# loicmagne/tinynerf

Measured on AMD Instinct MI355X. Metric: ray-samples/sec (K-Planes training step: sampler + render fwd + bwd + Adam), higher is better.
Workload: dtype f32 (f16x2-split products)

## Files before the change

tinynerf_amd/csrc/mlp_wgrad_rc.hip:

```cpp
#include "mlp_stage.h"
#include "mlp_f2_heads.h"
#include "b3_device.h"
#include "phase_timers.h"
#include <algorithm>

#ifndef TN_RC_SB
#define TN_RC_SB
#endif
TN_PHASE_COUNTERS(tn_phase_cycles_rc, tn_debug_phase_cycles_rc)
#define TN_PTR_BEGIN TN_PHASE_BEGIN(ptr_)
#define TN_PTR(k) TN_PHASE(tn_phase_cycles_rc, ptr_, k)
namespace {

using tn::f32x16;
using tn::f32x4;
using namespace tn::mlp;
namespace b3 = tn::b3;

constexpr int H = 64, NH = 4;

template <int CTRL>
__device__ __forceinline__ float dpp_max(float v) {
    return fmaxf(v, __int_as_float(__builtin_amdgcn_update_dpp(0, __float_as_int(v), CTRL, 0xf, 0xf, true)));
}
__device__ __forceinline__ float wave_max(float m) {
    m = dpp_max<0xB1>(m);
    m = dpp_max<0x4E>(m);
    m = dpp_max<0x141>(m);
    m = dpp_max<0x128>(m);
    const auto r16 = __builtin_amdgcn_permlane16_swap(__float_as_uint(m), __float_as_uint(m), false, false);
    m = fmaxf(__uint_as_float(r16[0]), __uint_as_float(r16[1]));
    const auto r32 = __builtin_amdgcn_permlane32_swap(__float_as_uint(m), __float_as_uint(m), false, false);
    return fmaxf(__uint_as_float(r32[0]), __uint_as_float(r32[1]));
}

__device__ __forceinline__ void load_block_f(const float *__restrict__ rows, int i, int h, float (&v)[16]) {
    const f32x4 *p = reinterpret_cast<const f32x4 *>(rows + i * 32 + 4 * h);
#pragma unroll
    for (int q = 0; q < 4; ++q) {
        const f32x4 t = p[2 * q];
        v[4 * q] = t[0]; v[4 * q + 1] = t[1]; v[4 * q + 2] = t[2]; v[4 * q + 3] = t[3];
    }
}

__device__ __forceinline__ void split_block(const float (&v)[16], b3::Op (&op)[2]) {
    const float a[8] = {v[0], v[1], v[2], v[3], v[4], v[5], v[6], v[7]};
    const float b[8] = {v[8], v[9], v[10], v[11], v[12], v[13], v[14], v[15]};
    op[0] = b3::split8(a);
    op[1] = b3::split8(b);
}

struct WOp { u32x4h a0h, a0l, a1h, a1l; };
__device__ __forceinline__ WOp load_w(const _Float16 *__restrict__ Wh, int plane, int stride, int j, int h, int b) {
    const _Float16 *p0 = Wh + j * stride + 16 * b + 8 * h, *p1 = p0 + 32 * stride;
    WOp w;
    w.a0h = *reinterpret_cast<const u32x4h *>(p0); w.a0l = *reinterpret_cast<const u32x4h *>(p0 + plane);
    w.a1h = *reinterpret_cast<const u32x4h *>(p1); w.a1l = *reinterpret_cast<const u32x4h *>(p1 + plane);
    return w;
}
template <bool S>
__device__ __forceinline__ void mma_sf(const WOp &w, const u32x4h &bh, const u32x4h &bl, f32x16 (&accS)[2], f32x16 (&accF)[2], bool first = false) {
    const f32x16 z = {0.f, 0.f, 0.f, 0.f, 0.f, 0.f, 0.f, 0.f, 0.f, 0.f, 0.f, 0.f, 0.f, 0.f, 0.f, 0.f};
    if constexpr (S) {
        accS[0] = mfma_f16(w.a0l, bh, first ? z : accS[0]);
        accS[1] = mfma_f16(w.a1l, bh, first ? z : accS[1]);
    }
    accF[0] = mfma_f16(bh, w.a0l, first ? z : accF[0]);
    accF[1] = mfma_f16(bh, w.a1l, first ? z : accF[1]);
    if constexpr (S) {
        accS[0] = mfma_f16(w.a0h, bl, accS[0]);
        accS[1] = mfma_f16(w.a1h, bl, accS[1]);
    }
    accF[0] = mfma_f16(bl, w.a0h, accF[0]);
    accF[1] = mfma_f16(bl, w.a1h, accF[1]);
    if constexpr (S) {
        accS[0] = mfma_f16(w.a0h, bh, accS[0]);
        accS[1] = mfma_f16(w.a1h, bh, accS[1]);
    }
    accF[0] = mfma_f16(bh, w.a0h, accF[0]);
    accF[1] = mfma_f16(bh, w.a1h, accF[1]);
}

struct RcArgs {
    MlpArgs a, b;
    const float *x, *aux;
    const float *ws_a, *ws_b;
    float *gW[5], *gB[5];
    float *gWs, *gBs;
    int64_t n;
};

template <int WPB, bool AUX, int OA, int OB, int NGA, int NBA>
__device__ __forceinline__ void wgrad_rc_body(const RcArgs &p, const float *__restrict__ ldsa, const float *__restrict__ ldsb, float *__restrict__ ,
                                              const float *__restrict__ px, const float *__restrict__ paux, const int *__restrict__ paidx,
                                              const float *__restrict__ pws_a, const float *__restrict__ pws_b)
{
    const int lane = tn::lane_id(), j_ = lane & 31, h_ = lane >> 5;
    const int wave = __builtin_amdgcn_readfirstlane(threadIdx.x >> 6);
    const int64_t n = p.n, n_tiles = (n + 31) >> 5;
    const int Rta = StashTile(H, NH, 0).rows(), Rtb = StashTile(H, 1, 0).rows();
    constexpr int nga = NGA, nba = NBA;
    constexpr bool has_aux = AUX;

    f32x16 acc[3][2][2];
#pragma unroll
    for (int l = 0; l < 3; ++l)
#pragma unroll
        for (int tn_ = 0; tn_ < 2; ++tn_)
#pragma unroll
            for (int tk = 0; tk < 2; ++tk)
#pragma unroll
                for (int r = 0; r < 16; ++r) acc[l][tn_][tk][r] = 0.0f;
    float db[3][2] = {{0.f, 0.f}, {0.f, 0.f}, {0.f, 0.f}};
    float dwo[OA][2], dws[OB][2], dbo[OA], dbs[OB];
#pragma unroll
    for (int o = 0; o < OA; ++o) { dwo[o][0] = dwo[o][1] = 0.f; dbo[o] = 0.f; }
#pragma unroll
    for (int o = 0; o < OB; ++o) { dws[o][0] = dws[o][1] = 0.f; dbs[o] = 0.f; }

    f32x4 fr[12], av[8];
    auto fetch_x = [&](int64_t t) {
        int64_t r = t * 32 + j_;
        r = r < n ? r : n - 1;
        const float *xr = px + r * 96 + 4 * h_;
#pragma unroll
        for (int g = 0; g < 12; ++g) fr[g] = *reinterpret_cast<const f32x4 *>(xr + 8 * g);
    };
    int aidx = 0;
    auto fetch_aidx = [&](int64_t t) {
        int64_t r = t * 32 + j_;
        r = r < n ? r : n - 1;
        if constexpr (has_aux) aidx = paidx[r];
    };
    auto fetch_aux = [&]() {
        if constexpr (has_aux) {
            const float *arow = paux + (int64_t)aidx * p.a.aux_stride + 4 * h_;
#pragma unroll
            for (int g = 0; g < 8; ++g) av[g] = *reinterpret_cast<const f32x4 *>(arow + 8 * (g < nga ? g : nga - 1));
        }
    };
    {
        const int64_t t0 = (int64_t)blockIdx.x * WPB + wave;
        fetch_aidx(t0 < n_tiles ? t0 : n_tiles - 1);
        fetch_aux();
        fetch_x(t0 < n_tiles ? t0 : n_tiles - 1);
    }
    float gqa[2][16], gqb[2][16];
    for (int64_t tile = (int64_t)blockIdx.x * WPB + wave; tile < n_tiles; tile += (int64_t)gridDim.x * WPB) {
        int j = j_, h = h_;
        asm volatile("" : "+v"(j), "+v"(h));
        const float *wsa = pws_a + tile * (int64_t)(Rta * 32);
        const float *wsb = pws_b + tile * (int64_t)(Rtb * 32);
        const _Float16 *W0 = reinterpret_cast<const _Float16 *>(ldsa + p.a.w_off[0]);
        const int plane0 = p.a.f2_plane[0], st0 = p.a.stride[0];
        const int64_t tile_next = tile + (int64_t)gridDim.x * WPB < n_tiles ? tile + (int64_t)gridDim.x * WPB : n_tiles - 1;
        fetch_aidx(tile_next);
        TN_PTR_BEGIN

        f32x16 accS[2], accF[2], actS[2], actF[2];
        if constexpr (has_aux) {
            WOp w = load_w(W0, plane0, st0, j, h, 6);
            float m = 0.0f;
#pragma unroll
            for (int g = 0; g < 8; ++g) m = tn::max_abs4(m, av[g]);
            float s_a, inv_a;
            f2_scales(wave_max(m), s_a, inv_a);
#pragma unroll
            for (int ba = 0; ba < nba; ++ba) {
                const WOp wn = load_w(W0, plane0, st0, j, h, 6 + (ba + 1 < nba ? ba + 1 : ba));
                const float v[8] = {av[2 * ba][0], av[2 * ba][1], av[2 * ba][2], av[2 * ba][3], av[2 * ba + 1][0], av[2 * ba + 1][1], av[2 * ba + 1][2], av[2 * ba + 1][3]};
                u32x4h bh, bl;
                f2_split8(v, s_a, bh, bl);
                mma_sf<true>(w, bh, bl, accS, accF, ba == 0);
                TN_RC_SB
                w = wn;
            }
            const float ca = inv_a * ldsa[p.a.f2_scale + 1];
#pragma unroll
            for (int ob = 0; ob < 2; ++ob) {
#pragma unroll
                for (int r = 0; r < 16; ++r) { actS[ob][r] = accS[ob][r] * ca; actF[ob][r] = accF[ob][r] * ca; }
            }
        } else {
            tn::zero_tiles(actS); tn::zero_tiles(actF);
        }
        TN_RC_SB
        TN_PTR(0)
        u32x4h xbh[6], xbl[6];
        float inv_x;
        {
            float m = 0.0f;
#pragma unroll
            for (int g = 0; g < 12; ++g) m = tn::max_abs4(m, fr[g]);
            float s_x;
            f2_scales(wave_max(m), s_x, inv_x);
#pragma unroll
            for (int b = 0; b < 6; ++b) {
                const float v[8] = {fr[2 * b][0], fr[2 * b][1], fr[2 * b][2], fr[2 * b][3], fr[2 * b + 1][0], fr[2 * b + 1][1], fr[2 * b + 1][2], fr[2 * b + 1][3]};
                f2_split8(v, s_x, xbh[b], xbl[b]);
            }
        }
        TN_RC_SB
        TN_PTR(1)
        load_block_f(wsa + (int64_t)((NH + 1) * H) * 32, j, h, gqa[0]);
        load_block_f(wsa + (int64_t)((NH + 1) * H + 32) * 32, j, h, gqa[1]);
        {
            WOp w = load_w(W0, plane0, st0, j, h, 0);
#pragma unroll
            for (int b = 0; b < 6; ++b) {
                const WOp wn = load_w(W0, plane0, st0, j, h, b + 1 < 6 ? b + 1 : b);
                mma_sf<true>(w, xbh[b], xbl[b], accS, accF, b == 0);
                TN_RC_SB
                w = wn;
            }
            const float cx = inv_x * ldsa[p.a.f2_scale + 1];
#pragma unroll
            for (int ob = 0; ob < 2; ++ob) {
                const f32x16 bias = tn::bias_tile(ldsa + p.a.b_off[0], ob, h);
                const float bl_ = ldsa[p.a.b_off[0] + 32 * ob + j];
#pragma unroll
                for (int r = 0; r < 16; ++r) {
                    actS[ob][r] = fmaf(accS[ob][r], cx, actS[ob][r]) + bias[r];
                    actF[ob][r] = fmaf(accF[ob][r], cx, actF[ob][r]) + bl_;
                }
                actS[ob] = tn::relu16(actS[ob]);
                actF[ob] = tn::relu16(actF[ob]);
            }
        }
        TN_RC_SB
        TN_PTR(2)
        {
            const _Float16 *W0s = reinterpret_cast<const _Float16 *>(ldsb + p.b.w_off[0]);
            const int pls = p.b.f2_plane[0], sts = p.b.stride[0];
            float gs[OB][16];
#pragma unroll
            for (int o = 0; o < OB; ++o) load_block_f(wsb + 2 * H * 32, o, h, gs[o]);
            WOp w = load_w(W0s, pls, sts, j, h, 0);
#pragma unroll
            for (int b = 0; b < 6; ++b) {
                const WOp wn = load_w(W0s, pls, sts, j, h, b + 1 < 6 ? b + 1 : b);
                mma_sf<false>(w, xbh[b], xbl[b], accS, accF, b == 0);
                TN_RC_SB
                w = wn;
            }
            const float c = inv_x * ldsb[p.b.f2_scale + 1];
#pragma unroll
            for (int ob = 0; ob < 2; ++ob) {
                const float bias = ldsb[p.b.b_off[0] + 32 * ob + j];
#pragma unroll
                for (int r = 0; r < 16; ++r) accF[ob][r] = fmaf(accF[ob][r], c, bias);
                accF[ob] = tn::relu16(accF[ob]);
            }
#pragma unroll
            for (int o = 0; o < OB; ++o) {
                float s0 = 0.f, s1 = 0.f, sg = 0.f;
#pragma unroll
                for (int r = 0; r < 16; ++r) { s0 = fmaf(gs[o][r], accF[0][r], s0); s1 = fmaf(gs[o][r], accF[1][r], s1); sg += gs[o][r]; }
                dws[o][0] += s0; dws[o][1] += s1; dbs[o] += sg;
            }
        }
        TN_RC_SB
        TN_PTR(3)

        float go[OA][16];
#pragma unroll
        for (int l = 1; l <= 3; ++l) {
            const _Float16 *Wl = reinterpret_cast<const _Float16 *>(ldsa + p.a.w_off[l]);
            const int plane = p.a.f2_plane[l], stride = p.a.stride[l];
            float (&gq)[2][16] = (l == 2) ? gqb : gqa;
            if (l < 3) {
                float (&gn)[2][16] = (l == 1) ? gqb : gqa;
                load_block_f(wsa + (int64_t)((NH + l + 1) * H) * 32, j, h, gn[0]);
                load_block_f(wsa + (int64_t)((NH + l + 1) * H + 32) * 32, j, h, gn[1]);
            }
            {
                b3::Op HB[2][2];
#pragma unroll
                for (int tk = 0; tk < 2; ++tk) {
                    float v[16];
#pragma unroll
                    for (int r = 0; r < 16; ++r) v[r] = actF[tk][r];
                    split_block(v, HB[tk]);
                }
#pragma unroll
                for (int tn_ = 0; tn_ < 2; ++tn_) {
                    float sg = 0.f;
#pragma unroll
                    for (int r = 0; r < 16; ++r) sg += gq[tn_][r];
                    db[l - 1][tn_] += sg;
                    b3::Op GA[2];
                    split_block(gq[tn_], GA);
#pragma unroll
                    for (int c = 0; c < 2; ++c)
#pragma unroll
                        for (int tk = 0; tk < 2; ++tk) acc[l - 1][tn_][tk] = b3::mfma6(GA[c], HB[tk][c], acc[l - 1][tn_][tk]);
                    TN_RC_SB
                }
            }
            TN_PTR(3 + l)
            if (l == 1) fetch_aux();
            if (l == 3) {
#pragma unroll
                for (int o = 0; o < OA; ++o) load_block_f(wsa + 2 * NH * H * 32, o, h, go[o]);
                fetch_x(tile_next);
            }
            WOp w = load_w(Wl, plane, stride, j, h, 0);
            float m = 0.0f;
#pragma unroll
            for (int kb = 0; kb < 2; ++kb)
#pragma unroll
                for (int r = 0; r < 16; ++r) m = fmaxf(m, actS[kb][r]);
            float s, inv;
            f2_scales(wave_max(m), s, inv);
#pragma unroll
            for (int b = 0; b < 4; ++b) {
                const WOp wn = load_w(Wl, plane, stride, j, h, b + 1 < 4 ? b + 1 : b);
                float v[8];
#pragma unroll
                for (int e = 0; e < 8; ++e) v[e] = actS[b >> 1][8 * (b & 1) + e];
                u32x4h bh, bl;
                f2_split8(v, s, bh, bl);
                if (l < 3) mma_sf<true>(w, bh, bl, accS, accF, b == 0);
                else mma_sf<false>(w, bh, bl, accS, accF, b == 0);
                TN_RC_SB
                w = wn;
            }
            const float c = inv * ldsa[p.a.f2_scale + 2 * l + 1];
#pragma unroll
            for (int ob = 0; ob < 2; ++ob) {
                const float bl_ = ldsa[p.a.b_off[l] + 32 * ob + j];
#pragma unroll
                for (int r = 0; r < 16; ++r) actF[ob][r] = fmaf(accF[ob][r], c, bl_);
                actF[ob] = tn::relu16(actF[ob]);
                if (l < 3) {
                    const f32x16 bias = tn::bias_tile(ldsa + p.a.b_off[l], ob, h);
#pragma unroll
                    for (int r = 0; r < 16; ++r) actS[ob][r] = fmaf(accS[ob][r], c, bias[r]);
                    actS[ob] = tn::relu16(actS[ob]);
                }
            }
            TN_RC_SB
            TN_PTR(6 + l)
        }
#pragma unroll
        for (int o = 0; o < OA; ++o) {
            float s0 = 0.f, s1 = 0.f, sg = 0.f;
#pragma unroll
            for (int r = 0; r < 16; ++r) { s0 = fmaf(go[o][r], actF[0][r], s0); s1 = fmaf(go[o][r], actF[1][r], s1); sg += go[o][r]; }
            dwo[o][0] += s0; dwo[o][1] += s1; dbo[o] += sg;
        }
        TN_PTR(10)
    }

    const int i = j_, h = h_;
#pragma unroll
    for (int l = 0; l < 3; ++l) {
#pragma unroll
        for (int tn_ = 0; tn_ < 2; ++tn_) {
#pragma unroll
            for (int tk = 0; tk < 2; ++tk) {
                tn::pin16(acc[l][tn_][tk]);
#pragma unroll
                for (int r = 0; r < 16; ++r) {
                    const int nn = 32 * tn_ + (r & 3) + 8 * (r >> 2) + 4 * h;
                    atomicAdd(&p.gW[l + 1][nn * H + 32 * tk + i], acc[l][tn_][tk][r]);
                }
            }
            float s = db[l][tn_];
            s += __shfl_xor(s, 32, 64);
            if (h == 0) atomicAdd(&p.gB[l + 1][32 * tn_ + i], s);
        }
    }
#pragma unroll
    for (int o = 0; o < OA; ++o) {
#pragma unroll
        for (int tk = 0; tk < 2; ++tk) {
            float s = dwo[o][tk];
            s += __shfl_xor(s, 32, 64);
            if (h == 0) atomicAdd(&p.gW[4][o * H + 32 * tk + i], s);
        }
        float s = dbo[o];
        s += __shfl_xor(s, 32, 64);
        if (lane == 0) atomicAdd(&p.gB[4][o], s);
    }
#pragma unroll
    for (int o = 0; o < OB; ++o) {
#pragma unroll
        for (int tk = 0; tk < 2; ++tk) {
            float s = dws[o][tk];
            s += __shfl_xor(s, 32, 64);
            if (h == 0) atomicAdd(&p.gWs[o * H + 32 * tk + i], s);
        }
        float s = dbs[o];
        s += __shfl_xor(s, 32, 64);
        if (lane == 0) atomicAdd(&p.gBs[o], s);
    }
}

template <int WPB, bool AUX, int OA, int OB, int NGA, int NBA>
__global__ __launch_bounds__(WPB * 64) void wgrad_rc_kernel(RcArgs p)
{
    extern __shared__ __attribute__((aligned(16))) float lds[];
    stage_weights_f2(p.a, lds);
    stage_weights_f2(p.b, lds + p.a.lds_floats);
    wgrad_rc_body<WPB, AUX, OA, OB, NGA, NBA>(p, lds, lds + p.a.lds_floats, nullptr, p.x, p.aux,
                                              p.a.aux_index, p.ws_a, p.ws_b);
}

struct FlArgs {
    const float *x, *aux;
    const int *aux_index;
    int aux_stride, pe, K0_a, K0_b;
    const float *ws_a, *ws_b;
    int rt_a, rt_b, g0_a, g0_b;
    float *gW0, *gB0, *gW0s, *gB0s;
    int64_t n;
};

constexpr int FL_RS = 36;
constexpr int FL_IN = 96, FL_AW = 56;
constexpr int FL_BUF = 128 * FL_RS + 32 * FL_IN + 32 * FL_AW;

__global__ __launch_bounds__(512) void wgrad_first_kernel(FlArgs p)
{
    extern __shared__ __attribute__((aligned(16))) float lds[];
    constexpr int NW = 8, NCH = 4;
    constexpr int g_chunks = 128 * 8, x_chunks = 32 * FL_IN / 4;
    const int lane = tn::lane_id(), i_ = lane & 31, h_ = lane >> 5;
    const int wave = __builtin_amdgcn_readfirstlane(threadIdx.x >> 6);
    const int64_t n = p.n, n_tiles = (n + 31) >> 5;
    const bool colour = wave < 5;
    const int tk = colour ? wave : wave - 5;
    f32x16 acc[2];
    float dbacc[2] = {0.f, 0.f};
#pragma unroll
    for (int m = 0; m < 2; ++m)
#pragma unroll
        for (int r = 0; r < 16; ++r) acc[m][r] = 0.0f;
    f32x4 pre[NCH];
    f32x4 preA = {0.f, 0.f, 0.f, 0.f};
    int aidx = 0;
    auto prefetch = [&](int64_t tile, int64_t tile_after) {
        const f32x4 *sa = reinterpret_cast<const f32x4 *>(p.ws_a + tile * (int64_t)p.rt_a * 32 + (int64_t)p.g0_a * 32);
        const f32x4 *sb = reinterpret_cast<const f32x4 *>(p.ws_b + tile * (int64_t)p.rt_b * 32 + (int64_t)p.g0_b * 32);
        const int64_t x0 = tile * 32 * (int64_t)FL_IN;
        const int64_t xlast = n * (int64_t)FL_IN - 4;
#pragma unroll
        for (int k = 0; k < NCH; ++k) {
            const int c = threadIdx.x + k * NW * 64;
            int64_t e = x0 + 4 * (int64_t)(c - g_chunks);
            e = e < 0 ? 0 : (e > xlast ? xlast : e);
            const f32x4 *px = reinterpret_cast<const f32x4 *>(p.x + e);
            const f32x4 *pg = c < 512 ? sa + c : sb + ((c - 512) & 511);
            pre[k] = *(c < g_chunks ? pg : px);
        }
        {
            const int s_ = (threadIdx.x >> 4) & 31, part = threadIdx.x & 15;
            preA = *reinterpret_cast<const f32x4 *>(p.aux + (int64_t)aidx * p.aux_stride + (4 * part < FL_AW ? 4 * part : 0));
            int64_t r_ = tile_after * 32 + s_;
            r_ = r_ < n ? r_ : n - 1;
            aidx = p.aux_index[r_];
        }
    };
    float *dummy = lds + 2 * FL_BUF;
    auto commit = [&](float *buf) {
        float *ldsX = buf + 128 * FL_RS, *ldsA = ldsX + 32 * FL_IN;
#pragma unroll
        for (int k = 0; k < NCH; ++k) {
            const int c = threadIdx.x + k * NW * 64;
            float *dst = c < g_chunks ? buf + (c >> 3) * FL_RS + (c & 7) * 4 : (c < g_chunks + x_chunks ? ldsX + 4 * (c - g_chunks) : dummy);
            *reinterpret_cast<f32x4 *>(dst) = pre[k];
        }
        const int s_ = threadIdx.x >> 4, part = threadIdx.x & 15;
        float *dst = 4 * part < FL_AW ? ldsA + s_ * FL_AW + 4 * part : dummy;
        *reinterpret_cast<f32x4 *>(dst) = preA;
    };
    const int64_t last = n_tiles - 1;
    int64_t tile = blockIdx.x;
    if (tile >= n_tiles) return;
    {
        int64_t r_ = tile * 32 + ((threadIdx.x >> 4) & 31);
        r_ = r_ < n ? r_ : n - 1;
        aidx = p.aux_index[r_];
    }
    {
        const int64_t t1 = tile + gridDim.x, t2 = t1 + gridDim.x;
        prefetch(tile, t1 < last ? t1 : last);
        commit(lds);
        __syncthreads();
        prefetch(t1 < last ? t1 : last, t2 < last ? t2 : last);
    }
    int cur = 0;
    for (; tile < n_tiles; tile += gridDim.x) {
        int i = i_, h = h_;
        asm volatile("" : "+v"(i), "+v"(h));
        float *buf = lds + cur * FL_BUF;
        float *nbuf = lds + (cur ^ 1) * FL_BUF;
        const int64_t t2 = tile + 2 * (int64_t)gridDim.x, t3 = t2 + gridDim.x;
        commit(nbuf);
        prefetch(t2 < last ? t2 : last, t3 < last ? t3 : last);
        const float *ldsX = buf + 128 * FL_RS, *ldsA = ldsX + 32 * FL_IN;
        {
            const int grow = colour ? 0 : 64;
            const f32x4 *g0 = reinterpret_cast<const f32x4 *>(buf + (grow + i) * FL_RS + 16 * h);
            const f32x4 *g1 = reinterpret_cast<const f32x4 *>(buf + (grow + 32 + i) * FL_RS + 16 * h);
            const int q = 32 * tk + i;
            const bool xcol = q < FL_IN;
            const int ac = q - FL_IN < FL_AW ? q - FL_IN : FL_AW - 1;
            const float *cp = xcol ? ldsX + 16 * h * FL_IN + q : ldsA + 16 * h * FL_AW + (ac < 0 ? 0 : ac);
            const int cstride = xcol ? FL_IN : FL_AW;
            float gs0 = 0.f, gs1 = 0.f;
#pragma unroll
            for (int c = 0; c < 2; ++c) {
                const f32x4 ga = g0[2 * c], gb = g0[2 * c + 1], gc = g1[2 * c], gd = g1[2 * c + 1];
                float xv[8];
#pragma unroll
                for (int u = 0; u < 8; ++u) xv[u] = cp[(8 * c + u) * cstride];
                const float v0[8] = {ga[0], ga[1], ga[2], ga[3], gb[0], gb[1], gb[2], gb[3]};
                const float v1[8] = {gc[0], gc[1], gc[2], gc[3], gd[0], gd[1], gd[2], gd[3]};
                const b3::Op XB = b3::split8(xv);
                acc[0] = b3::mfma6(b3::split8(v0), XB, acc[0]);
                acc[1] = b3::mfma6(b3::split8(v1), XB, acc[1]);
                gs0 += ((ga[0] + ga[1]) + (ga[2] + ga[3])) + ((gb[0] + gb[1]) + (gb[2] + gb[3]));
                gs1 += ((gc[0] + gc[1]) + (gc[2] + gc[3])) + ((gd[0] + gd[1]) + (gd[2] + gd[3]));
            }
            if (tk == 0) { dbacc[0] += gs0; dbacc[1] += gs1; }
        }
        __syncthreads();
        cur ^= 1;
    }
    const int i = i_, h = h_;
    const int q = 32 * tk + i;
    int col; bool ok;
    float *gW; int ldw;
    if (colour) { gW = p.gW0; ldw = p.K0_a; ok = q < FL_IN || q - FL_IN < p.pe; col = q < FL_IN ? p.pe + q : q - FL_IN; }
    else { gW = p.gW0s; ldw = p.K0_b; ok = true; col = q; }
#pragma unroll
    for (int m = 0; m < 2; ++m) {
        tn::pin16(acc[m]);
#pragma unroll
        for (int r = 0; r < 16; ++r) {
            const int nn = 32 * m + (r & 3) + 8 * (r >> 2) + 4 * h;
            if (ok) atomicAdd(&gW[(int64_t)nn * ldw + col], acc[m][r]);
        }
        if (tk == 0) {
            float s = dbacc[m];
            s += __shfl_xor(s, 32, 64);
            if (h == 0) atomicAdd(&(colour ? p.gB0 : p.gB0s)[32 * m + i], s);
        }
    }
}

}

static bool lean_pair_ok(const tn_mlp_desc *d, const tn_mlp_desc *p)
{
    const bool f2 = (d->flags & TN_MLP_F16X2) && (p->flags & TN_MLP_F16X2);
    return f2 && d->n_layers == 5 && p->n_layers == 2 && d->in_dim == 96 && p->in_dim == 96 && d->encoding == TN_ENC_AUX_CAT &&
           p->encoding == TN_ENC_NONE && d->dims[0] == 147 && d->dims[1] == 64 && d->dims[2] == 64 && d->dims[3] == 64 &&
           d->dims[4] == 64 && d->dims[5] == 3 && p->dims[0] == 96 && p->dims[1] == 64 && p->dims[2] == 1 &&
           d->aux_stride >= FL_AW && (d->aux_stride & 3) == 0;
}

extern "C" int tn_mlp_lean_supported(const tn_mlp_desc *desc, const tn_mlp_desc *partner)
{
    return desc && partner && lean_pair_ok(desc, partner);
}

static int lean_plan(RcArgs &p, const tn_mlp_desc *desc, const tn_mlp_desc *partner, const float *x, const float *aux, int64_t n,
                     float *const *gw, float *const *gb, float *const *gws, float *const *gbs, const float *ws_a, const float *ws_b)
{
    TN_REQUIRE(desc && partner && x && gw && gb && gws && gbs && ws_a && ws_b, TN_E_NULL, "tn_mlp_wgrad_lean_pair: null pointer");
    int Ha = 0, Hb = 0;
    if (int rc = plan(desc, p.a, Ha)) return rc;
    if (int rc = plan(partner, p.b, Hb)) return rc;
    TN_REQUIRE(lean_pair_ok(desc, partner), TN_E_CONFIG, "TN_MLP_LEAN: the reference's decoders (run.py:133-139) as f16x2 heads (TN_MLP_F16X2): "
                                                         "colour 147 -> 64 x 4 -> 3 on [per-ray table (51), x (96)], sigma 96 -> 64 -> 1");
    TN_REQUIRE(aux && ((uintptr_t)aux & 15) == 0 && p.a.aux_index, TN_E_NULL, "TN_MLP_LEAN: aux table (16-byte aligned) and aux_index are required");
    TN_REQUIRE((((uintptr_t)x | (uintptr_t)ws_a | (uintptr_t)ws_b) & 15) == 0, TN_E_ALIGN, "TN_MLP_LEAN: x / workspaces must be 16-byte aligned");
    if (n <= 0) return TN_OK;
    for (int l = 0; l < 5; ++l) TN_REQUIRE(gw[l] && gb[l], TN_E_NULL, "TN_MLP_LEAN: null gradient pointer");
    TN_REQUIRE(gws[0] && gbs[0] && gws[1] && gbs[1], TN_E_NULL, "TN_MLP_LEAN: null gradient pointer");
    plan_f2(p.a, 64);
    plan_f2(p.b, 64);
    TN_REQUIRE(((size_t)p.a.lds_floats + (size_t)p.b.lds_floats) * 4 <= (size_t)LDS_LIMIT_BYTES, TN_E_CONFIG, "TN_MLP_LEAN: weights do not fit LDS");
    return TN_OK;
}

extern "C" __attribute__((visibility("hidden"))) int tn_mlp_wgrad_lean_check(const tn_mlp_desc *desc, const tn_mlp_desc *partner, const float *x,
                                                                             const float *aux, int64_t n, float *const *gw, float *const *gb,
                                                                             float *const *gws, float *const *gbs, const float *ws_a,
                                                                             const float *ws_b)
{
    RcArgs p;
    return lean_plan(p, desc, partner, x, aux, n, gw, gb, gws, gbs, ws_a, ws_b);
}

extern "C" int tn_mlp_wgrad_lean_pair(const tn_mlp_desc *desc, const tn_mlp_desc *partner, const float *x, const float *aux, int64_t n,
                                      float *const *gw, float *const *gb, float *const *gws, float *const *gbs, const float *ws_a,
                                      const float *ws_b, void *stream)
{
    RcArgs p;
    if (int rc = lean_plan(p, desc, partner, x, aux, n, gw, gb, gws, gbs, ws_a, ws_b)) return rc;
    if (n <= 0) return TN_OK;
    hipStream_t s = (hipStream_t)stream;
    FlArgs f;
    f.x = x; f.aux = aux; f.aux_index = p.a.aux_index; f.aux_stride = p.a.aux_stride;
    f.pe = p.a.K0 - p.a.in_dim;
    f.ws_a = ws_a; f.ws_b = ws_b;
    f.rt_a = StashTile(H, NH, 0).rows(); f.rt_b = StashTile(H, 1, 0).rows();
    f.g0_a = NH * H; f.g0_b = H;
    f.K0_a = p.a.K0; f.K0_b = p.b.K0;
    f.gW0 = gw[0]; f.gB0 = gb[0]; f.gW0s = gws[0]; f.gB0s = gbs[0];
    f.n = n;
    const size_t lds1 = (2 * (size_t)FL_BUF + 16) * 4;
    if (int rc = launch(wgrad_first_kernel, 8, lds1, grid_blocks(n, 1, 256 * 2), s, "wgrad_first_kernel", f)) return rc;
    p.x = x; p.aux = aux; p.ws_a = ws_a; p.ws_b = ws_b; p.n = n;
    for (int l = 0; l < 5; ++l) { p.gW[l] = gw[l]; p.gB[l] = gb[l]; }
    p.gWs = gws[1]; p.gBs = gbs[1];
    constexpr int WPB = 4;
    const size_t lds_bytes = ((size_t)p.a.lds_floats + (size_t)p.b.lds_floats) * 4;
    return launch(wgrad_rc_kernel<WPB, true, 3, 1, 7, 4>, WPB, lds_bytes, grid_blocks(n, WPB, 256), s, "wgrad_rc_kernel", p);
}
```

Before: 346.0 million.

## Restructure first-layer weight-gradient kernel with specialized waves and run-length aux reduction

Rewrites the first-layer weight-gradient kernel into warp-specialized roles. Four waves run the MFMA products over the 96 input columns for both heads. One wave computes the aux-table columns by summing gradients over runs of samples that share the same aux index, replacing per-sample MFMA work on gathered aux rows. A loader wave prefetches the stashed gradients and also accumulates the density-head bias. Partial accumulators from the two k-halves are combined through LDS before the atomics, which halves the atomic traffic. Risks: the run-length path is serial per wave and depends on sorted or clustered aux indices, and the kernel now hardcodes pe=51 and 32-bit tile counts.

```diff
diff --git a/tinynerf_amd/csrc/mlp_wgrad_rc.hip b/tinynerf_amd/csrc/mlp_wgrad_rc.hip
--- a/tinynerf_amd/csrc/mlp_wgrad_rc.hip
+++ b/tinynerf_amd/csrc/mlp_wgrad_rc.hip
@@ -418,136 +418,207 @@
 };
 
 constexpr int FL_RS = 36;
-constexpr int FL_IN = 96, FL_AW = 56;
-constexpr int FL_BUF = 128 * FL_RS + 32 * FL_IN + 32 * FL_AW;
-
-__global__ __launch_bounds__(512) void wgrad_first_kernel(FlArgs p)
-{
-    extern __shared__ __attribute__((aligned(16))) float lds[];
-    constexpr int NW = 8, NCH = 4;
-    constexpr int g_chunks = 128 * 8, x_chunks = 32 * FL_IN / 4;
-    const int lane = tn::lane_id(), i_ = lane & 31, h_ = lane >> 5;
-    const int wave = __builtin_amdgcn_readfirstlane(threadIdx.x >> 6);
-    const int64_t n = p.n, n_tiles = (n + 31) >> 5;
-    const bool colour = wave < 5;
-    const int tk = colour ? wave : wave - 5;
-    f32x16 acc[2];
-    float dbacc[2] = {0.f, 0.f};
-#pragma unroll
-    for (int m = 0; m < 2; ++m)
-#pragma unroll
-        for (int r = 0; r < 16; ++r) acc[m][r] = 0.0f;
-    f32x4 pre[NCH];
-    f32x4 preA = {0.f, 0.f, 0.f, 0.f};
-    int aidx = 0;
-    auto prefetch = [&](int64_t tile, int64_t tile_after) {
-        const f32x4 *sa = reinterpret_cast<const f32x4 *>(p.ws_a + tile * (int64_t)p.rt_a * 32 + (int64_t)p.g0_a * 32);
-        const f32x4 *sb = reinterpret_cast<const f32x4 *>(p.ws_b + tile * (int64_t)p.rt_b * 32 + (int64_t)p.g0_b * 32);
-        const int64_t x0 = tile * 32 * (int64_t)FL_IN;
-        const int64_t xlast = n * (int64_t)FL_IN - 4;
-#pragma unroll
-        for (int k = 0; k < NCH; ++k) {
-            const int c = threadIdx.x + k * NW * 64;
-            int64_t e = x0 + 4 * (int64_t)(c - g_chunks);
-            e = e < 0 ? 0 : (e > xlast ? xlast : e);
-            const f32x4 *px = reinterpret_cast<const f32x4 *>(p.x + e);
-            const f32x4 *pg = c < 512 ? sa + c : sb + ((c - 512) & 511);
-            pre[k] = *(c < g_chunks ? pg : px);
-        }
-        {
-            const int s_ = (threadIdx.x >> 4) & 31, part = threadIdx.x & 15;
-            preA = *reinterpret_cast<const f32x4 *>(p.aux + (int64_t)aidx * p.aux_stride + (4 * part < FL_AW ? 4 * part : 0));
-            int64_t r_ = tile_after * 32 + s_;
-            r_ = r_ < n ? r_ : n - 1;
-            aidx = p.aux_index[r_];
-        }
-    };
-    float *dummy = lds + 2 * FL_BUF;
-    auto commit = [&](float *buf) {
-        float *ldsX = buf + 128 * FL_RS, *ldsA = ldsX + 32 * FL_IN;
-#pragma unroll
-        for (int k = 0; k < NCH; ++k) {
-            const int c = threadIdx.x + k * NW * 64;
-            float *dst = c < g_chunks ? buf + (c >> 3) * FL_RS + (c & 7) * 4 : (c < g_chunks + x_chunks ? ldsX + 4 * (c - g_chunks) : dummy);
-            *reinterpret_cast<f32x4 *>(dst) = pre[k];
-        }
-        const int s_ = threadIdx.x >> 4, part = threadIdx.x & 15;
-        float *dst = 4 * part < FL_AW ? ldsA + s_ * FL_AW + 4 * part : dummy;
-        *reinterpret_cast<f32x4 *>(dst) = preA;
-    };
-    const int64_t last = n_tiles - 1;
-    int64_t tile = blockIdx.x;
-    if (tile >= n_tiles) return;
-    {
-        int64_t r_ = tile * 32 + ((threadIdx.x >> 4) & 31);
-        r_ = r_ < n ? r_ : n - 1;
-        aidx = p.aux_index[r_];
-    }
-    {
-        const int64_t t1 = tile + gridDim.x, t2 = t1 + gridDim.x;
-        prefetch(tile, t1 < last ? t1 : last);
-        commit(lds);
-        __syncthreads();
-        prefetch(t1 < last ? t1 : last, t2 < last ? t2 : last);
-    }
-    int cur = 0;
-    for (; tile < n_tiles; tile += gridDim.x) {
-        int i = i_, h = h_;
-        asm volatile("" : "+v"(i), "+v"(h));
-        float *buf = lds + cur * FL_BUF;
-        float *nbuf = lds + (cur ^ 1) * FL_BUF;
-        const int64_t t2 = tile + 2 * (int64_t)gridDim.x, t3 = t2 + gridDim.x;
-        commit(nbuf);
-        prefetch(t2 < last ? t2 : last, t3 < last ? t3 : last);
-        const float *ldsX = buf + 128 * FL_RS, *ldsA = ldsX + 32 * FL_IN;
-        {
-            const int grow = colour ? 0 : 64;
-            const f32x4 *g0 = reinterpret_cast<const f32x4 *>(buf + (grow + i) * FL_RS + 16 * h);
-            const f32x4 *g1 = reinterpret_cast<const f32x4 *>(buf + (grow + 32 + i) * FL_RS + 16 * h);
-            const int q = 32 * tk + i;
-            const bool xcol = q < FL_IN;
-            const int ac = q - FL_IN < FL_AW ? q - FL_IN : FL_AW - 1;
-            const float *cp = xcol ? ldsX + 16 * h * FL_IN + q : ldsA + 16 * h * FL_AW + (ac < 0 ? 0 : ac);
-            const int cstride = xcol ? FL_IN : FL_AW;
-            float gs0 = 0.f, gs1 = 0.f;
-#pragma unroll
-            for (int c = 0; c < 2; ++c) {
-                const f32x4 ga = g0[2 * c], gb = g0[2 * c + 1], gc = g1[2 * c], gd = g1[2 * c + 1];
-                float xv[8];
-#pragma unroll
-                for (int u = 0; u < 8; ++u) xv[u] = cp[(8 * c + u) * cstride];
-                const float v0[8] = {ga[0], ga[1], ga[2], ga[3], gb[0], gb[1], gb[2], gb[3]};
-                const float v1[8] = {gc[0], gc[1], gc[2], gc[3], gd[0], gd[1], gd[2], gd[3]};
-                const b3::Op XB = b3::split8(xv);
-                acc[0] = b3::mfma6(b3::split8(v0), XB, acc[0]);
-                acc[1] = b3::mfma6(b3::split8(v1), XB, acc[1]);
-                gs0 += ((ga[0] + ga[1]) + (ga[2] + ga[3])) + ((gb[0] + gb[1]) + (gb[2] + gb[3]));
-                gs1 += ((gc[0] + gc[1]) + (gc[2] + gc[3])) + ((gd[0] + gd[1]) + (gd[2] + gd[3]));
-            }
-            if (tk == 0) { dbacc[0] += gs0; dbacc[1] += gs1; }
-        }
-        __syncthreads();
-        cur ^= 1;
-    }
-    const int i = i_, h = h_;
-    const int q = 32 * tk + i;
-    int col; bool ok;
-    float *gW; int ldw;
-    if (colour) { gW = p.gW0; ldw = p.K0_a; ok = q < FL_IN || q - FL_IN < p.pe; col = q < FL_IN ? p.pe + q : q - FL_IN; }
-    else { gW = p.gW0s; ldw = p.K0_b; ok = true; col = q; }
-#pragma unroll
-    for (int m = 0; m < 2; ++m) {
-        tn::pin16(acc[m]);
+constexpr int FL_IN = 96, FL_PE = 51;
+constexpr int FL_AW = 56;
+constexpr int FL_NW = 6;
+constexpr int FL_BUF = 128 * FL_RS + 32 * FL_IN;
+constexpr int FL_PARK = 2 * 6 * 1024;
+constexpr int FL_LDS = std::max(2 * FL_BUF, FL_PARK + 64 * FL_PE);
+
+__device__ __forceinline__ void fl_park3(float *__restrict__ park, int m, const f32x16 (&a)[3], int lane) {
+#pragma unroll
+    for (int tk = 0; tk < 3; ++tk)
+#pragma unroll
+        for (int r = 0; r < 16; ++r) park[(3 * m + tk) * 1024 + 64 * r + lane] = a[tk][r];
+}
+__device__ __forceinline__ void fl_flush3(const float *__restrict__ park, int m, f32x16 (&a)[3], int lane, float *__restrict__ gW, int ldw, int col0) {
+    const int i = lane & 31, h = lane >> 5;
+#pragma unroll
+    for (int tk = 0; tk < 3; ++tk) {
+        tn::pin16(a[tk]);
 #pragma unroll
         for (int r = 0; r < 16; ++r) {
             const int nn = 32 * m + (r & 3) + 8 * (r >> 2) + 4 * h;
-            if (ok) atomicAdd(&gW[(int64_t)nn * ldw + col], acc[m][r]);
-        }
-        if (tk == 0) {
-            float s = dbacc[m];
-            s += __shfl_xor(s, 32, 64);
-            if (h == 0) atomicAdd(&(colour ? p.gB0 : p.gB0s)[32 * m + i], s);
-        }
+            atomicAdd(&gW[(int64_t)nn * ldw + col0 + 32 * tk + i], a[tk][r] + park[(3 * m + tk) * 1024 + 64 * r + lane]);
+        }
+    }
+}
+
+__global__ __launch_bounds__(FL_NW * 64, 3) void wgrad_first_kernel(FlArgs p)
+{
+    extern __shared__ __attribute__((aligned(16))) float lds[];
+    const int lane = tn::lane_id(), i_ = lane & 31;
+    const int wave = __builtin_amdgcn_readfirstlane(threadIdx.x >> 6);
+    const int64_t n = p.n;
+    const int n_tiles = (int)((n + 31) >> 5), last = n_tiles - 1;
+    const int tile0 = blockIdx.x;
+    if (tile0 >= n_tiles) return;
+    const int G_ = gridDim.x;
+    using S0 = std::integral_constant<int, 0>;
+    using S1 = std::integral_constant<int, 1>;
+    auto at = [&](int t) { return t < last ? t : last; };
+    auto tiles = [&](auto &&prefetch, auto &&commit, auto &&work) {
+        prefetch(tile0, tile0, S0());
+        commit(lds, S0());
+        prefetch(at(tile0 + G_), at(tile0 + G_), S0());
+        prefetch(-1, at(tile0 + 2 * G_), S1());
+        __syncthreads();
+        auto step = [&](int tile, auto S) {
+            constexpr int s_ = decltype(S)::value;
+            commit(lds + (s_ ^ 1) * FL_BUF, S);
+            prefetch(at(tile + 2 * G_), at(tile + 3 * G_), S);
+            work(lds + s_ * FL_BUF, at(tile + G_));
+            __syncthreads();
+        };
+        for (int tile = tile0; tile < n_tiles; tile += 2 * G_) {
+            step(tile, S0());
+            if (tile + G_ < n_tiles) step(tile + G_, S1());
+        }
+    };
+    float *park = lds;
+    if (wave < 4) {
+        const int head = wave >> 1, kh = wave & 1;
+        f32x16 acc[2][3];
+#pragma unroll
+        for (int m = 0; m < 2; ++m)
+#pragma unroll
+            for (int tk = 0; tk < 3; ++tk)
+#pragma unroll
+                for (int r = 0; r < 16; ++r) acc[m][tk][r] = 0.0f;
+        auto none = [](auto...) {};
+        tiles(none, none, [&](const float *buf, int64_t) {
+            int l = lane;
+            asm volatile("" : "+v"(l));
+            const int i = l & 31, h = l >> 5;
+            const int ks = 16 * kh + 8 * h;
+            b3::Op GA[2];
+#pragma unroll
+            for (int m = 0; m < 2; ++m) {
+                const f32x4 *g = reinterpret_cast<const f32x4 *>(buf + (64 * head + 32 * m + i) * FL_RS + ks);
+                const f32x4 ga = g[0], gb = g[1];
+                const float v[8] = {ga[0], ga[1], ga[2], ga[3], gb[0], gb[1], gb[2], gb[3]};
+                GA[m] = b3::split8(v);
+            }
+            const float *cp = buf + 128 * FL_RS + ks * FL_IN + i;
+#pragma unroll
+            for (int tk = 0; tk < 3; ++tk) {
+                float xv[8];
+#pragma unroll
+                for (int u = 0; u < 8; ++u) xv[u] = cp[u * FL_IN + 32 * tk];
+                const b3::Op XB = b3::split8(xv);
+                acc[0][tk] = b3::mfma6(GA[0], XB, acc[0][tk]);
+                acc[1][tk] = b3::mfma6(GA[1], XB, acc[1][tk]);
+            }
+        });
+        float *pk = park + head * 6 * 1024;
+        float *gW = head == 0 ? p.gW0 : p.gW0s;
+        const int ldw = head == 0 ? p.K0_a : p.K0_b, col0 = head == 0 ? FL_PE : 0;
+        if (kh == 0) fl_park3(pk, 1, acc[1], lane); else fl_park3(pk, 0, acc[0], lane);
+        __syncthreads();
+        if (kh == 0) fl_flush3(pk, 0, acc[0], lane, gW, ldw, col0); else fl_flush3(pk, 1, acc[1], lane, gW, ldw, col0);
+    } else if (wave == 4) {
+        float racc[FL_PE];
+#pragma unroll
+        for (int c = 0; c < FL_PE; ++c) racc[c] = 0.0f;
+        float dbc = 0.0f;
+        auto fetch_idx = [&](int64_t tile) {
+            int64_t r = tile * 32 + i_;
+            r = r < n ? r : n - 1;
+            return p.aux_index[r];
+        };
+        int vidx = fetch_idx(tile0);
+        typedef const float __attribute__((address_space(4))) *ConstRow;
+        const ConstRow table = reinterpret_cast<ConstRow>(reinterpret_cast<uintptr_t>(p.aux));
+        const int64_t astride = p.aux_stride;
+        f32x4 pre[12];
+        auto prefetch = [&](int64_t t1, int64_t, auto) {
+            if (t1 < 0) return;
+            const float *xb = p.x + t1 * (int64_t)(32 * FL_IN);
+            const int rem = (int)std::min<int64_t>((n - t1 * 32) * FL_IN - 4, 32 * FL_IN);
+#pragma unroll
+            for (int k = 0; k < 12; ++k) pre[k] = *reinterpret_cast<const f32x4 *>(xb + std::min(4 * lane + 256 * k, rem));
+        };
+        auto commit = [&](float *buf, auto) {
+            float *dx = buf + 128 * FL_RS + 4 * lane;
+#pragma unroll
+            for (int k = 0; k < 12; ++k) *reinterpret_cast<f32x4 *>(dx + 256 * k) = pre[k];
+        };
+        tiles(prefetch, commit, [&](const float *buf, int64_t tile_next) {
+            const int vnext = fetch_idx(tile_next);
+            float g[32];
+            {
+                const f32x4 *gp = reinterpret_cast<const f32x4 *>(buf + lane * FL_RS);
+#pragma unroll
+                for (int q = 0; q < 8; ++q) {
+                    const f32x4 t = gp[q];
+                    g[4 * q] = t[0]; g[4 * q + 1] = t[1]; g[4 * q + 2] = t[2]; g[4 * q + 3] = t[3];
+                }
+            }
+            const int vprev = __shfl_up(vidx, 1, 64);
+            const unsigned opens = (unsigned)__ballot(vidx != vprev);
+            float row[FL_PE];
+            auto open_run = [&](int s) {
+                const ConstRow t = table + (int64_t)__builtin_amdgcn_readlane(vidx, s) * astride;
+#pragma unroll
+                for (int c = 0; c < FL_PE; ++c) row[c] = t[c];
+            };
+            float S = 0.0f;
+            auto close_run = [&]() {
+#pragma unroll
+                for (int c = 0; c < FL_PE; ++c) racc[c] = fmaf(S, row[c], racc[c]);
+                dbc += S;
+            };
+            open_run(0);
+#pragma unroll
+            for (int s = 0; s < 32; ++s) {
+                if (s > 0 && ((opens >> s) & 1u)) {
+                    close_run();
+                    S = 0.0f;
+                    open_run(s);
+                }
+                S += g[s];
+            }
+            close_run();
+            vidx = vnext;
+        });
+        float *tr = park + FL_PARK;
+#pragma unroll
+        for (int c = 0; c < FL_PE; ++c) tr[lane * FL_PE + c] = racc[c];
+        __syncthreads();
+#pragma unroll 3
+        for (int it = 0; it < FL_PE; ++it) {
+            const int e = 64 * it + lane, f = e / FL_PE;
+            atomicAdd(&p.gW0[(int64_t)f * p.K0_a + (e - f * FL_PE)], tr[e]);
+        }
+        atomicAdd(&p.gB0[lane], dbc);
+    } else {
+        f32x4 pre[2][16];
+        auto prefetch = [&](int64_t, int64_t tile, auto S) {
+            constexpr int s_ = decltype(S)::value;
+            const f32x4 *sa = reinterpret_cast<const f32x4 *>(p.ws_a + tile * (int64_t)p.rt_a * 32 + (int64_t)p.g0_a * 32) + lane;
+            const f32x4 *sb = reinterpret_cast<const f32x4 *>(p.ws_b + tile * (int64_t)p.rt_b * 32 + (int64_t)p.g0_b * 32) + lane;
+#pragma unroll
+            for (int k = 0; k < 8; ++k) { pre[s_][k] = sa[64 * k]; pre[s_][8 + k] = sb[64 * k]; }
+        };
+        auto commit = [&](float *buf, auto S) {
+            constexpr int s_ = decltype(S)::value;
+            float *dst = buf + (lane >> 3) * FL_RS + (lane & 7) * 4;
+#pragma unroll
+            for (int k = 0; k < 16; ++k) *reinterpret_cast<f32x4 *>(dst + 8 * k * FL_RS) = pre[s_][k];
+        };
+        float dbs = 0.0f;
+        tiles(prefetch, commit, [&](const float *buf, int64_t) {
+            const f32x4 *sp = reinterpret_cast<const f32x4 *>(buf + (64 + lane) * FL_RS);
+            float ss = 0.0f;
+#pragma unroll
+            for (int q = 0; q < 8; ++q) {
+                const f32x4 u = sp[q];
+                ss += (u[0] + u[1]) + (u[2] + u[3]);
+            }
+            dbs += ss;
+        });
+        __syncthreads();
+        atomicAdd(&p.gB0s[lane], dbs);
     }
 }
 
@@ -613,8 +684,10 @@
     f.K0_a = p.a.K0; f.K0_b = p.b.K0;
     f.gW0 = gw[0]; f.gB0 = gb[0]; f.gW0s = gws[0]; f.gB0s = gbs[0];
     f.n = n;
-    const size_t lds1 = (2 * (size_t)FL_BUF + 16) * 4;
-    if (int rc = launch(wgrad_first_kernel, 8, lds1, grid_blocks(n, 1, 256 * 2), s, "wgrad_first_kernel", f)) return rc;
+    TN_REQUIRE(n < ((int64_t)1 << 35), TN_E_CONFIG, "TN_MLP_LEAN: more than 2^35 samples");
+    TN_REQUIRE(f.pe == FL_PE, TN_E_CONFIG, "TN_MLP_LEAN: the colour head's first layer takes 51 table columns");
+    const size_t lds1 = (size_t)FL_LDS * 4;
+    if (int rc = launch(wgrad_first_kernel, FL_NW, lds1, grid_blocks(n, 1, 256 * 2), s, "wgrad_first_kernel", f)) return rc;
     p.x = x; p.aux = aux; p.ws_a = ws_a; p.ws_b = ws_b; p.n = n;
     for (int l = 0; l < 5; ++l) { p.gW[l] = gw[l]; p.gB[l] = gb[l]; }
     p.gWs = gws[1]; p.gBs = gbs[1];
```

New measurement: 348.7 million, median of 6. No clear change (+0.8%).

## Deepen wgrad_first prefetch to a three-buffer LDS ring with two register stages

Applied to the files above, without the earlier changes.

Converts the first-layer weight-gradient kernel from a double-buffered LDS scheme with one register prefetch stage to a three-slot LDS ring fed by two alternating register stages. Global loads are issued four tiles ahead, which gives more time to hide memory latency. Because LDS per block grows to about 113 KB, the grid cap is halved to match the lower residency. The trade is fewer resident blocks and more registers held for prefetch in exchange for deeper latency hiding.

```diff
diff --git a/tinynerf_amd/csrc/mlp_wgrad_rc.hip b/tinynerf_amd/csrc/mlp_wgrad_rc.hip
--- a/tinynerf_amd/csrc/mlp_wgrad_rc.hip
+++ b/tinynerf_amd/csrc/mlp_wgrad_rc.hip
@@ -420,6 +420,7 @@
 constexpr int FL_RS = 36;
 constexpr int FL_IN = 96, FL_AW = 56;
 constexpr int FL_BUF = 128 * FL_RS + 32 * FL_IN + 32 * FL_AW;
+constexpr int FL_RING = 3;
 
 __global__ __launch_bounds__(512) void wgrad_first_kernel(FlArgs p)
 {
@@ -437,10 +438,12 @@
     for (int m = 0; m < 2; ++m)
 #pragma unroll
         for (int r = 0; r < 16; ++r) acc[m][r] = 0.0f;
-    f32x4 pre[NCH];
-    f32x4 preA = {0.f, 0.f, 0.f, 0.f};
-    int aidx = 0;
-    auto prefetch = [&](int64_t tile, int64_t tile_after) {
+    struct Stage { f32x4 pre[NCH]; f32x4 preA; int aidx; };
+    Stage st0, st1;
+    auto prefetch = [&](Stage &st, int64_t tile, int64_t tile_after) {
+        f32x4 (&pre)[NCH] = st.pre;
+        f32x4 &preA = st.preA;
+        int &aidx = st.aidx;
         const f32x4 *sa = reinterpret_cast<const f32x4 *>(p.ws_a + tile * (int64_t)p.rt_a * 32 + (int64_t)p.g0_a * 32);
         const f32x4 *sb = reinterpret_cast<const f32x4 *>(p.ws_b + tile * (int64_t)p.rt_b * 32 + (int64_t)p.g0_b * 32);
         const int64_t x0 = tile * 32 * (int64_t)FL_IN;
@@ -462,43 +465,45 @@
             aidx = p.aux_index[r_];
         }
     };
-    float *dummy = lds + 2 * FL_BUF;
-    auto commit = [&](float *buf) {
+    float *dummy = lds + FL_RING * FL_BUF;
+    auto commit = [&](const Stage &st, float *buf) {
         float *ldsX = buf + 128 * FL_RS, *ldsA = ldsX + 32 * FL_IN;
 #pragma unroll
         for (int k = 0; k < NCH; ++k) {
             const int c = threadIdx.x + k * NW * 64;
             float *dst = c < g_chunks ? buf + (c >> 3) * FL_RS + (c & 7) * 4 : (c < g_chunks + x_chunks ? ldsX + 4 * (c - g_chunks) : dummy);
-            *reinterpret_cast<f32x4 *>(dst) = pre[k];
+            *reinterpret_cast<f32x4 *>(dst) = st.pre[k];
         }
         const int s_ = threadIdx.x >> 4, part = threadIdx.x & 15;
         float *dst = 4 * part < FL_AW ? ldsA + s_ * FL_AW + 4 * part : dummy;
-        *reinterpret_cast<f32x4 *>(dst) = preA;
+        *reinterpret_cast<f32x4 *>(dst) = st.preA;
     };
-    const int64_t last = n_tiles - 1;
+    const int64_t last = n_tiles - 1, grid = gridDim.x;
     int64_t tile = blockIdx.x;
     if (tile >= n_tiles) return;
-    {
-        int64_t r_ = tile * 32 + ((threadIdx.x >> 4) & 31);
+    auto clamped = [&](int64_t t) { return t < last ? t : last; };
+    auto first_index = [&](int64_t t) {
+        int64_t r_ = t * 32 + ((threadIdx.x >> 4) & 31);
         r_ = r_ < n ? r_ : n - 1;
-        aidx = p.aux_index[r_];
-    }
-    {
-        const int64_t t1 = tile + gridDim.x, t2 = t1 + gridDim.x;
-        prefetch(tile, t1 < last ? t1 : last);
-        commit(lds);
-        __syncthreads();
-        prefetch(t1 < last ? t1 : last, t2 < last ? t2 : last);
-    }
+        return p.aux_index[r_];
+    };
+    st0.aidx = first_index(tile);
+    st1.aidx = first_index(clamped(tile + grid));
+    prefetch(st0, tile, clamped(tile + 2 * grid));
+    prefetch(st1, clamped(tile + grid), clamped(tile + 3 * grid));
+    commit(st0, lds);
+    prefetch(st0, clamped(tile + 2 * grid), clamped(tile + 4 * grid));
+    commit(st1, lds + FL_BUF);
+    prefetch(st1, clamped(tile + 3 * grid), clamped(tile + 5 * grid));
+    __syncthreads();
     int cur = 0;
-    for (; tile < n_tiles; tile += gridDim.x) {
+    auto step = [&](Stage &st) {
         int i = i_, h = h_;
         asm volatile("" : "+v"(i), "+v"(h));
         float *buf = lds + cur * FL_BUF;
-        float *nbuf = lds + (cur ^ 1) * FL_BUF;
-        const int64_t t2 = tile + 2 * (int64_t)gridDim.x, t3 = t2 + gridDim.x;
-        commit(nbuf);
-        prefetch(t2 < last ? t2 : last, t3 < last ? t3 : last);
+        float *nbuf = lds + (cur == 0 ? 2 : cur - 1) * FL_BUF;
+        commit(st, nbuf);
+        prefetch(st, clamped(tile + 4 * grid), clamped(tile + 6 * grid));
         const float *ldsX = buf + 128 * FL_RS, *ldsA = ldsX + 32 * FL_IN;
         {
             const int grow = colour ? 0 : 64;
@@ -527,8 +532,15 @@
             if (tk == 0) { dbacc[0] += gs0; dbacc[1] += gs1; }
         }
         __syncthreads();
-        cur ^= 1;
-    }
+        cur = cur == FL_RING - 1 ? 0 : cur + 1;
+        tile += grid;
+    };
+    const int64_t steps = (last - tile) / grid + 1;
+    for (int64_t k = 0; k < steps / 2; ++k) {
+        step(st0);
+        step(st1);
+    }
+    if (steps & 1) step(st0);
     const int i = i_, h = h_;
     const int q = 32 * tk + i;
     int col; bool ok;
@@ -613,8 +625,8 @@
     f.K0_a = p.a.K0; f.K0_b = p.b.K0;
     f.gW0 = gw[0]; f.gB0 = gb[0]; f.gW0s = gws[0]; f.gB0s = gbs[0];
     f.n = n;
-    const size_t lds1 = (2 * (size_t)FL_BUF + 16) * 4;
-    if (int rc = launch(wgrad_first_kernel, 8, lds1, grid_blocks(n, 1, 256 * 2), s, "wgrad_first_kernel", f)) return rc;
+    const size_t lds1 = (FL_RING * (size_t)FL_BUF + 16) * 4;
+    if (int rc = launch(wgrad_first_kernel, 8, lds1, grid_blocks(n, 1, 256), s, "wgrad_first_kernel", f)) return rc;
     p.x = x; p.aux = aux; p.ws_a = ws_a; p.ws_b = ws_b; p.n = n;
     for (int l = 0; l < 5; ++l) { p.gW[l] = gw[l]; p.gB[l] = gb[l]; }
     p.gWs = gws[1]; p.gBs = gbs[1];
```

New measurement: 354.1 million before, 353.3 million after. Within noise of the previous version (-0.2%).
